# ViktorLiang/GW-Depth

Hardware: AMD Instinct MI355X
Metric: images/sec (train fwd+bwd) 480x640 bs=8/GPU (higher is better)
Workload: dtype bf16; 1 GPU; GW-Depth full model (res50 + DETR 6+6 + 4-scale ReferTransformer + decoder) fwd+17 losses+bwd+clip+AdamW, 480x640, bs=8/GPU, dropout 0.1; global_batch=8, parallelism=dp1, launch=hipgraph, graph_segments=1, grad_buckets=8

## Files before the change

gw_depth_amd/hip.py:

```python
import ctypes
import os

import torch

_HERE = os.path.dirname(os.path.abspath(__file__))
LIB_PATH = os.environ.get("GWD_LIB") or os.path.join(_HERE, "libgwdepth_hip.so")

F32, BF16 = 0, 1
ACT_NONE, ACT_RELU, ACT_GELU, ACT_ELU, ACT_SIGMOID = 0, 1, 2, 3, 4
WS_INORM_GELU, WS_RESAMPLE_BWD, WS_EVAL, WS_PLANE, WS_HEALTH = 0, 1, 2, 3, 4
GATHER_CONV, GATHER_TRANSPOSED, GATHER_UPSAMPLED = 0, 1, 2
RESAMPLE_BILINEAR_AC, RESAMPLE_NEAREST = 0, 1

ENTRY_POINTS = [
    "gwd_version", "gwd_arch", "gwd_conv_forward", "gwd_conv_wgrad", "gwd_weight_prep", "gwd_act_backward",
    "gwd_colsum", "gwd_layernorm_forward", "gwd_layernorm_backward", "gwd_softmax_forward",
    "gwd_softmax_backward", "gwd_silog_sums", "gwd_silog_backward", "gwd_seg_ce_sum", "gwd_seg_ce_backward",
    "gwd_sqnorm", "gwd_adamw_step", "gwd_resample_forward", "gwd_resample_backward", "gwd_avgpool_forward",
    "gwd_avgpool_backward", "gwd_winattn_forward", "gwd_winattn_backward", "gwd_tokattn_forward",
    "gwd_tokattn_backward", "gwd_tokattn_pair_forward", "gwd_tokattn_pair_backward", "gwd_upsample_taps_collapse", "gwd_upsample_taps_fold", "gwd_certain_sample", "gwd_lsap", "gwd_window_map", "gwd_window_map_multi",
    "gwd_inorm_gelu_forward", "gwd_inorm_gelu_backward", "gwd_weight_prep_batch",
    "gwd_point_sample_forward", "gwd_point_sample_backward", "gwd_act_backward_colsum", "gwd_resample_backward_sep",
    "gwd_softmax_masked_forward", "gwd_softmax_scaled_backward", "gwd_query_workspace", "gwd_eval_accumulate", "gwd_colsum_batch", "gwd_conv_wgrad_batch",
    "gwd_conv_wgrad_takes_bias",
    "gwd_plane_loss_forward", "gwd_plane_loss_backward", "gwd_collate",
    "gwd_anchor_depth_forward", "gwd_anchor_depth_backward", "gwd_mha_flash_forward", "gwd_mha_flash_backward",
    "gwd_ref_scores_forward", "gwd_ref_scores_backward", "gwd_ref_mix_forward", "gwd_ref_mix_backward", "gwd_unpad_add_batch", "gwd_stem_pack", "gwd_stem_forward", "gwd_pos_sine", "gwd_silog_finalize", "gwd_psp_pool_forward", "gwd_psp_pool_backward",
    "gwd_match_cost", "gwd_set_losses_forward", "gwd_set_losses_backward", "gwd_set_losses_focal_forward", "gwd_set_losses_focal_backward", "gwd_resample_u8_pass", "gwd_gather2d", "gwd_point_sample_backward_gather", "gwd_point_sample_framed_forward", "gwd_point_sample_framed_backward", "gwd_stride_place", "gwd_color_adjust", "gwd_bmm",
    "gwd_dense_postprocess", "gwd_line_postprocess", "gwd_line_score",
    "gwd_dense_postprocess_resized",
    "gwd_resample_u8_pass_batch", "gwd_gather2d_batch", "gwd_color_adjust_batch",
    "gwd_pyr_tail_forward", "gwd_pyr_tail_backward", "gwd_pyr_tail_fold_wgrad",
    "gwd_widen_u16_batch",
    "gwd_line_nms",
    "gwd_eval_frames",
    "gwd_segment_stats", "gwd_health_decide", "gwd_adamw_step_guarded",
    "gwd_adamw_step_ema", "gwd_ema_swap",
]


class HipUnavailable(RuntimeError):
    pass


class ConvDesc(ctypes.Structure):
    _fields_ = [("x", ctypes.c_void_p), ("w", ctypes.c_void_p), ("y", ctypes.c_void_p), ("z", ctypes.c_void_p),
                ("scale", ctypes.c_void_p), ("shift", ctypes.c_void_p), ("residual", ctypes.c_void_p),
                ("zero_page", ctypes.c_void_p), ("mult", ctypes.c_void_p), ("gate", ctypes.c_void_p)] + \
               [(n, ctypes.c_int32) for n in ("B", "Hi", "Wi", "Cin", "Ho", "Wo", "Cout", "KH", "KW", "stride", "pad",
                                              "gather", "Hv", "Wv", "act")] + \
               [("act_scale", ctypes.c_float), ("dtype", ctypes.c_int32), ("gate_act", ctypes.c_int32),
                ("ln_mean", ctypes.c_void_p), ("ln_rstd", ctypes.c_void_p), ("ln_C", ctypes.c_int32), ("reserved", ctypes.c_int32),
                ("dbias", ctypes.c_void_p)]


class BmmDesc(ctypes.Structure):
    _fields_ = [("a", ctypes.c_void_p), ("b", ctypes.c_void_p), ("c", ctypes.c_void_p)] + \
               [(n, ctypes.c_int64) for n in ("a_sb0", "a_sb1", "a_ld", "b_sb0", "b_sb1", "b_ld", "c_sb0", "c_sb1", "c_ld")] + \
               [(n, ctypes.c_int32) for n in ("M", "N", "K", "nb0", "nb1", "a_kmajor", "b_kmajor", "c_is_f32_accumulate", "splits")] + \
               [("alpha", ctypes.c_float), ("dtype", ctypes.c_int32)]


class PrepJob(ctypes.Structure):
    _fields_ = [("w", ctypes.c_void_p), ("row_scale", ctypes.c_void_p), ("w_fwd", ctypes.c_void_p), ("w_dgrad", ctypes.c_void_p),
                ("N", ctypes.c_int32), ("taps", ctypes.c_int32), ("C", ctypes.c_int32), ("block0", ctypes.c_int32),
                ("Np", ctypes.c_int32), ("Cg", ctypes.c_int32), ("Cgp", ctypes.c_int32), ("reserved", ctypes.c_int32)]


class UnpadJob(ctypes.Structure):
    _fields_ = [("src", ctypes.c_void_p), ("dst", ctypes.c_void_p), ("N", ctypes.c_int32), ("taps", ctypes.c_int32), ("G", ctypes.c_int32),
# ... 145 lines not shown
        L.gwd_set_losses_forward.argtypes = [vp] * 9 + [f32] + [vp] * 4 + [i32] * 6 + [vp]
        L.gwd_set_losses_backward.argtypes = [vp] * 8 + [f32] + [vp] * 6 + [i32] * 6 + [vp]
        L.gwd_set_losses_focal_forward.argtypes = [vp] * 9 + [f32] * 2 + [vp] * 4 + [i32] * 6 + [vp]
        L.gwd_set_losses_focal_backward.argtypes = [vp] * 8 + [f32] * 2 + [vp] * 6 + [i32] * 6 + [vp]
        L.gwd_color_adjust.argtypes = [vp, vp, vp, i64, i32, f32, vp]
        L.gwd_bmm.argtypes = [ctypes.POINTER(BmmDesc), vp]
        L.gwd_stride_place.argtypes = [vp, vp, vp] + [i32] * 8 + [vp]
        L.gwd_psp_pool_forward.argtypes = [vp] * 5 + [i32] * 5 + [vp]
        L.gwd_psp_pool_backward.argtypes = [vp] * 6 + [i32] * 6 + [vp]
        L.gwd_pos_sine.argtypes = [vp, vp, vp, vp, vp, i32, i32, i32, i32, i32, i32, i32, vp]
        L.gwd_stem_pack.argtypes = [vp, vp, vp, vp]
        L.gwd_stem_forward.argtypes = [vp, vp, vp, vp, i32, i32, i32, i32, vp]
        L.gwd_softmax_forward.argtypes = [vp, vp, i64, i32, i32, vp]
        L.gwd_softmax_backward.argtypes = [vp, vp, vp, i64, i32, i32, vp]
        L.gwd_silog_sums.argtypes = [vp, vp, vp, i32, i32, i32, i32, i32, i32, i32, vp]
        L.gwd_silog_backward.argtypes = [vp, vp, vp, vp, f32, f32, vp, i32, i32, i32, i32, i32, i32, i32, vp]
        L.gwd_seg_ce_sum.argtypes = [vp, vp, vp, i64, i32, vp]
        L.gwd_seg_ce_backward.argtypes = [vp, vp, vp, f32, vp, i64, i32, vp]
        L.gwd_resample_forward.argtypes = [vp, vp] + [i32] * 9 + [vp]
        L.gwd_resample_backward.argtypes = [vp, vp] + [i32] * 7 + [vp, i32, i32, vp]
        L.gwd_avgpool_forward.argtypes = [vp, vp] + [i32] * 6 + [vp]
        L.gwd_avgpool_backward.argtypes = [vp, vp] + [i32] * 6 + [vp]
        sp = ctypes.POINTER(Strided)
        L.gwd_winattn_forward.argtypes = [sp, sp, sp, sp, vp, vp, i32, vp, i64, i32, i32, i32, f32, i32, vp]
        L.gwd_winattn_backward.argtypes = [sp] * 7 + [vp, vp, vp, i32, vp, i64, i32, i32, i32, f32, i32, i32, vp]
        L.gwd_ref_scores_forward.argtypes = [sp, vp, vp, i32, i32, i32, i32, i32, f32, i32, vp]
        L.gwd_ref_scores_backward.argtypes = [sp, vp, vp, sp, vp, i32, i32, i32, i32, i32, f32, i32, vp]
        L.gwd_ref_mix_forward.argtypes = [vp, vp, vp, vp, i32, i32, i32, i32, i32, i32, vp]
        L.gwd_ref_mix_backward.argtypes = [vp, vp, vp, vp, vp, i32, i32, i32, i32, i32, i32, vp]
        L.gwd_tokattn_forward.argtypes = [sp] * 4 + [i64, i32, i32, f32, i32, vp]
        L.gwd_tokattn_backward.argtypes = [sp] * 7 + [i64, i32, i32, f32, i32, vp]
        L.gwd_upsample_taps_collapse.argtypes = [vp, vp, i32, i32, i32, vp]
        L.gwd_upsample_taps_fold.argtypes = [vp, vp, i32, i32, vp]
        L.gwd_tokattn_pair_forward.argtypes = [sp] * 6 + [i64, i32, i32, f32, i32, vp]
        L.gwd_tokattn_pair_backward.argtypes = [sp] * 10 + [i64, i32, i32, f32, i32, vp]
        L.gwd_certain_sample.argtypes = [vp, vp, vp, i32, i32, i32, i32, i32, vp, i32, i32, vp]
        L.gwd_lsap.argtypes = [vp, vp, vp, i32, i32, i32, i32, i32, vp]
        L.gwd_inorm_gelu_forward.argtypes = [vp, vp, vp, vp, vp, i64, i64, i32, i32, ctypes.c_float, i32, vp]
        L.gwd_inorm_gelu_backward.argtypes = [vp, vp, vp, vp, vp, i64, i64, i32, i32, i32, vp]
        L.gwd_query_workspace.argtypes = [i32, ctypes.POINTER(ctypes.c_int64), i32]
        L.gwd_query_workspace.restype = ctypes.c_int64
        L.gwd_eval_accumulate.argtypes = [vp, vp, vp, i64, i64, i64, vp, vp, vp, vp, vp, i32, i64, f32, f32, i32, i32, vp]
        L.gwd_dense_postprocess.argtypes = [vp, vp, i64, i64, i64, vp, vp, vp, vp, i32, i32, i32, f32, f32, i32, i32, vp]
        L.gwd_dense_postprocess_resized.argtypes = [vp, vp, i64, i64, i64, vp, vp, i32, vp, vp, vp] + [i32] * 5 + [f32, f32, i32, i32, vp]
        L.gwd_line_postprocess.argtypes = [vp] * 7 + [i32, i32, i32, f32, vp]
        dp = ctypes.POINTER(ctypes.c_double)
        L.gwd_line_score.argtypes = [vp] * 5 + [dp, i32, dp, i32] + [vp] * 4 + [i32] * 4 + [i64, i64, vp]
        L.gwd_softmax_masked_forward.argtypes = [vp, vp, vp, i64, i32, i64, ctypes.c_float, i32, vp]
        L.gwd_softmax_scaled_backward.argtypes = [vp, vp, vp, i64, i32, ctypes.c_float, i32, vp]
        L.gwd_resample_backward_sep.argtypes = [vp, vp, vp] + [i32] * 9 + [vp]
        L.gwd_act_backward_colsum.argtypes = [vp, vp, vp, vp, i64, i32, i32, ctypes.c_float, vp, i32, vp]
        L.gwd_point_sample_forward.argtypes = [vp, vp, vp, i32, i32, i32, i32, i32, i32, i32, vp]
        L.gwd_point_sample_backward.argtypes = [vp, vp, vp, i32, i32, i32, i32, i32, i32, i32, vp]
        L.gwd_point_sample_backward_gather.argtypes = [vp, vp, vp, i32, i32, i32, i32, i32, i32, i32, vp]
        L.gwd_point_sample_framed_forward.argtypes = [vp, vp, vp, i32, i32, i32, i32, i32, i32, i32, i32, i32, vp]
        L.gwd_point_sample_framed_backward.argtypes = [vp, vp, vp, i32, i32, i32, i32, i32, i32, i32, i32, i32, vp]
        L.gwd_weight_prep_batch.argtypes = [vp, i32, i32, vp, vp]
        L.gwd_window_map.argtypes = [vp, vp, vp, i32, i32, i32, i32, i32, i32, i32, vp]
        L.gwd_window_map_multi.argtypes = [vp, vp, vp, vp, i32, i32, i32, i32, i32, i32, i32, vp]
        L.gwd_sqnorm.argtypes = [vp, vp, i64, vp]
        L.gwd_adamw_step.argtypes = [vp, vp, vp, vp, vp, vp, i64] + [f32] * 9 + [vp]
        pvp, pi32 = ctypes.POINTER(ctypes.c_void_p), ctypes.POINTER(ctypes.c_int32)
        L.gwd_pyr_tail_forward.argtypes = [vp, pvp, pi32, pi32, i32] + [vp] * 6 + [i32] * 6 + [vp]
        L.gwd_pyr_tail_backward.argtypes = [vp, pvp, pi32, pi32, i32] + [i32] * 5 + [vp]
        L.gwd_pyr_tail_fold_wgrad.argtypes = [vp, pvp, i32, vp, i32, i32, i32, vp]
        L.gwd_widen_u16_batch.argtypes = [ctypes.POINTER(WidenJob), i32, vp]
# ... 482 lines not shown
                                                 dtype_code(ra), self._stream(ra, ref_v, q_new, att)), "gwd_ref_mix_forward")

    def ref_mix_backward(self, att, ref_v, g, d_ra, d_ref_v, H):
        B, T, R = att.shape[0], att.shape[1], att.shape[2]
        self._check(self.lib.gwd_ref_mix_backward(_ptr(att), _ptr(ref_v), _ptr(g), _ptr(d_ra), _ptr(d_ref_v), B, T, R, H,
                                                  ref_v.shape[2] // H, dtype_code(att), self._stream(att, ref_v, g, d_ra, d_ref_v)),
                    "gwd_ref_mix_backward")

    def tokattn_forward(self, q, k, v, o, scale):
        W, N, H, _ = q.shape
        s = [_strided(t) for t in (q, k, v, o)]
        self._check(self.lib.gwd_tokattn_forward(*[ctypes.byref(x) for x in s], W, H, k.shape[3], scale, dtype_code(q),
                                                 self._stream(q, k, v, o)), "gwd_tokattn_forward")

    def tokattn_backward(self, q, k, v, go, gq, gk, gv, scale):
        W, N, H, _ = q.shape
        s = [_strided(t) for t in (q, k, v, go, gq, gk, gv)]
        self._check(self.lib.gwd_tokattn_backward(*[ctypes.byref(x) for x in s], W, H, k.shape[3], scale, dtype_code(q),
                                                  self._stream(q, go, gq)), "gwd_tokattn_backward")

    def upsample_taps_collapse(self, w, wk):
        Cout, KH, KW, Cin = w.shape
        if (KH, KW) != (3, 3) or tuple(wk.shape) != (Cin, 4, 4, Cout) or w.dtype != torch.float32 or not (w.is_contiguous() and wk.is_contiguous()):
            raise ValueError("upsample_taps_collapse: w (Cout,3,3,Cin) fp32 -> wk (Cin,4,4,Cout), both contiguous")
        self._check(self.lib.gwd_upsample_taps_collapse(_ptr(w), _ptr(wk), Cout, Cin, dtype_code(wk), self._stream(w, wk)), "gwd_upsample_taps_collapse")

    def upsample_taps_fold(self, D, dw):
        Cout, KH, KW, Cin = dw.shape
        if (KH, KW) != (3, 3) or tuple(D.shape) != (Cin, 4, 4, Cout) or D.dtype != torch.float32 or dw.dtype != torch.float32 \
                or not (D.is_contiguous() and dw.is_contiguous()):
            raise ValueError("upsample_taps_fold: D (Cin,4,4,Cout) fp32 -> dw (Cout,3,3,Cin) fp32, both contiguous")
        self._check(self.lib.gwd_upsample_taps_fold(_ptr(D), _ptr(dw), Cout, Cin, self._stream(D, dw)), "gwd_upsample_taps_fold")

    PYR_MAX_BRANCHES = 4

    @staticmethod
    def _pyr_branches(maps, B, N, like):
        if not 1 <= len(maps) <= HipLibrary.PYR_MAX_BRANCHES:
            raise ValueError("pyr_tail: 1 to %d low-resolution branches, got %d" % (HipLibrary.PYR_MAX_BRANCHES, len(maps)))
        for m in maps:
            if m.dim() != 5 or m.shape[0] != B or m.shape[3] != 9 or m.shape[4] != N or m.dtype != like.dtype or not m.is_contiguous():
                raise ValueError("pyr_tail: a product map is (B,h,w,9,N) contiguous in the map's dtype, got %r" % (tuple(m.shape),))
        ptrs = (ctypes.c_void_p * len(maps))(*[m.data_ptr() for m in maps])
        hk = (ctypes.c_int32 * len(maps))(*[m.shape[1] for m in maps])
        wk = (ctypes.c_int32 * len(maps))(*[m.shape[2] for m in maps])
        return ptrs, hk, wk

    def pyr_tail_forward(self, part, Zs, gamma, beta, z, y, mean, rstd, gelu):
        B, H, W, N = part.shape
        ptrs, hk, wk = self._pyr_branches(Zs, B, N, part)
        rc = self.lib.gwd_pyr_tail_forward(_ptr(part), ptrs, hk, wk, len(Zs), _ptr(gamma), _ptr(beta), _ptr(z), _ptr(y), _ptr(mean), _ptr(rstd),
                                           B, H, W, N, int(bool(gelu)), dtype_code(part), self._stream(part, y, *Zs))
        if rc == -4:
            return False
        self._check(rc, "gwd_pyr_tail_forward")
        return True

    def pyr_tail_backward(self, gz, Gs):
        B, H, W, N = gz.shape
        ptrs, hk, wk = self._pyr_branches(Gs, B, N, gz)
        self._check(self.lib.gwd_pyr_tail_backward(_ptr(gz), ptrs, hk, wk, len(Gs), B, H, W, N, dtype_code(gz), self._stream(gz, *Gs)),
                    "gwd_pyr_tail_backward")

    def pyr_tail_fold_wgrad(self, d_hi, d_low, dw, C2):
        N, Cw, nlow = dw.shape[0], dw.shape[-1], len(d_low)
        nbr = Cw // C2 - 1
# ... 309 lines not shown
```

gw_depth_amd/ops.py:

```python
import bisect
import os

import torch
import torch.nn.functional as F

from . import hip
from .hip import (ACT_ELU, ACT_GELU, ACT_NONE, ACT_RELU, ACT_SIGMOID, GATHER_CONV, GATHER_TRANSPOSED,
                  GATHER_UPSAMPLED)

__all__ = ["conv2d", "linear", "layer_norm", "softmax_lastdim", "silog_loss", "seg_cross_entropy",
           "ACT_NONE", "ACT_RELU", "ACT_GELU", "ACT_ELU", "ACT_SIGMOID"]


def _lib():
    return hip.library()


class WeightCache:

    def __init__(self, persistent=(), frozen=False):
        self.frozen = bool(frozen)
        self._derived = {}
        self.ranges = sorted((int(a), int(b)) for a, b in persistent)
        self._starts, self._ends, self._merged_from = [], [], -1
# ... 246 lines not shown
    N, C = w.shape[0], w.shape[-1]
    _lib().weight_prep(w.detach(), row_scale, out, None, N, w.numel() // (N * C), C, hip.F32 if dtype == torch.float32 else hip.BF16)
    return out


def derived_weight(w, tag, make):
    if _ACTIVE_WEIGHTS is not None and _ACTIVE_WEIGHTS.frozen and w.is_cuda and not torch.is_grad_enabled():
        return _ACTIVE_WEIGHTS.derived(w, tag, make)
    return make()


def _weight_transposed(w, row_scale, dtype):
    if dtype == torch.bfloat16 and _ACTIVE_WEIGHTS is not None:
        cached = _ACTIVE_WEIGHTS.get(w, row_scale, "t")
        if cached is not None:
            return cached
    N, C = w.shape[0], w.shape[-1]
    taps = w.numel() // (N * C)
    out = torch.empty((C,) + tuple(w.shape[1:-1]) + (N,), dtype=dtype, device=w.device)
    _lib().weight_prep(w.detach(), row_scale, None, out, N, taps, C, hip.F32 if dtype == torch.float32 else hip.BF16)
    return out


_DIM_T = {}


def _upsampled_dgrad_weight(w, dtype):
    Cout, _, _, Cin = w.shape
    wk = torch.empty((Cin, 4, 4, Cout), dtype=dtype, device=w.device)
    _lib().upsample_taps_collapse(w.detach().float().contiguous(), wk)
    return wk




def mask_levels(pad_mask, sizes):
    lib = _lib()
    B = pad_mask.shape[0]
    full = pad_mask.contiguous().view(torch.uint8) if pad_mask.dtype == torch.bool else pad_mask.contiguous()
    out = []
    for h, w in sizes:
        lvl = torch.empty((B, h, w), dtype=torch.uint8, device=pad_mask.device)
        counts = torch.empty((B, h, w, 2), dtype=torch.int16, device=pad_mask.device)
        lib.pos_counts(full, lvl, counts)
        m = lvl.view(torch.bool)
        m._gwd_counts = counts
        out.append(m)
    return out


def pos_sine(mask, num_pos_feats, normalize, temperature=10000.0):
    counts = mask._gwd_counts
    key = (num_pos_feats, float(temperature), str(mask.device))
    dim_t = _DIM_T.get(key)
    if dim_t is None:
        t = torch.arange(num_pos_feats, dtype=torch.float32, device=mask.device)
        dim_t = _DIM_T[key] = temperature ** (2 * torch.div(t, 2, rounding_mode="floor") / num_pos_feats)
    B, h, w, _ = counts.shape
    out = torch.empty((B, h, w, 2 * num_pos_feats), dtype=torch.float32, device=mask.device)
    _lib().pos_emit(counts, dim_t, out, normalize)
    return out


_STEM_PACKED = {}
_STEM_RETIRED = []

# ... 117 lines not shown
        dims, pad, geom, sink = ctx.cfg
        gx, gw = _conv_backward_stride1(ctx.needs_input_grad[0], ctx.needs_input_grad[1], x, w, gy.contiguous(), g_in, dims, pad, geom, sink)
        return gx, gw, None, None, None, None


def conv2d_padded(x, w, pad, geom, fanout=False):
    return _PadConvFn.apply(x, w, int(pad), tuple(int(v) for v in geom), _sink(w), bool(fanout))


class _ConvFn(torch.autograd.Function):

    @staticmethod
    def forward(ctx, x, w, bias, residual, row_scale, shift_const, stride, pad, act, act_scale, virt, shadow, sinks, mult=None, fanout=False,
                in_gate=ACT_NONE, defer=False, gate_src=None):
        lib = _lib()
        ctx.fan = bool(fanout)
        ctx.in_gate, ctx.defer = int(in_gate), bool(defer)
        if defer and (act not in (ACT_RELU, ACT_ELU, ACT_GELU) or act_scale != 1.0 or mult is not None or (act == ACT_GELU and fanout)):
            raise ValueError("conv2d: defer needs ReLU / ELU / GELU with act_scale 1 and no dropout multiplier")
        if in_gate not in (ACT_NONE, ACT_RELU, ACT_ELU, ACT_GELU) or (in_gate == ACT_GELU) != (gate_src is not None):
            raise ValueError("conv2d: in_gate is ReLU or ELU, or GELU with the producer's pre-activation tensor as gate_src")
        B, Hi, Wi, Cin = x.shape
        Cout, KH, KW, Cw = w.shape
        if Cw != Cin:
            raise ValueError("conv2d: weight expects %d input channels, input has %d" % (Cw, Cin))
        if virt is None:
            Ho = (Hi + 2 * pad - KH) // stride + 1
            Wo = (Wi + 2 * pad - KW) // stride + 1
            gather, vv = GATHER_CONV, (0, 0)
        else:
            Ho, Wo = virt[0] + 2 * pad - KH + 1, virt[1] + 2 * pad - KW + 1
            gather, vv = GATHER_UPSAMPLED, tuple(virt)
        x = x.contiguous()
        wk = _weight_for(w, row_scale, x.dtype, shadow)
        shift = shift_const if bias is None else (bias.detach().float() if shift_const is None else shift_const + bias.detach().float())
        y = torch.empty((B, Ho, Wo, Cout), dtype=x.dtype, device=x.device)
        need_grad = any(ctx.needs_input_grad[:4])
        z = torch.empty_like(y) if (act == ACT_GELU and need_grad) else None
        if residual is not None:
            residual = residual.contiguous()
        dims = (B, Hi, Wi, Cin, Ho, Wo, Cout, KH, KW)
        if mult is not None:
            mult = mult.contiguous()
        lib.conv_forward(x, wk, y, dims, z=z, shift=shift, residual=residual, stride=stride, pad=pad, gather=gather,
                         virt=vv, act=act, act_scale=act_scale, mult=mult)
        ctx.cfg = (dims, stride, pad, act, act_scale, gather, vv, bias is not None, residual is not None)
        ctx.sinks = sinks
        if mult is not None and (act not in (ACT_NONE, ACT_RELU) or (act == ACT_RELU and residual is not None)):
            raise ValueError("conv2d: a dropout multiplier is supported behind no activation (+ skip) or behind ReLU (no skip) only")
        ctx.save_for_backward(x, w, row_scale, z if act == ACT_GELU else (y if act != ACT_NONE else None), mult, gate_src)
        if defer and act == ACT_GELU:
            if z is None:
                z = y
            ctx.mark_non_differentiable(z)
            ctx.set_materialize_grads(False)
            return y, z
        if fanout:
            return y, x.view_as(x)
        return y

    @staticmethod
    def backward(ctx, gy, *g_fan):
        if gy is None:
            return (None,) * 18
        g_in = _fan_in(ctx, g_fan)
        x, w, row_scale, ref, mult, gate_src = ctx.saved_tensors
        dims, stride, pad, act, act_scale, gather, vv, has_bias, has_res = ctx.cfg
        gy = gy.contiguous()
        w_sink, b_sink = ctx.sinks if ctx.sinks is not None else (None, None)
        want_b = has_bias and ctx.needs_input_grad[2]
        dv, bias_done = _conv_act_backward(gy, ref, mult, act, act_scale, ctx.defer, b_sink if want_b else None, dims)
        gx = g_in
        if ctx.needs_input_grad[0]:
            gx = _conv_dgrad(x, w, row_scale, dv, g_in, dims, stride, pad, gather, vv, ctx.in_gate, gate_src)
        gw, gb = _conv_param_grads(x, w, row_scale, dv, dims, stride, pad, gather, vv, ctx.needs_input_grad[1], want_b and not bias_done,
                                   w_sink, b_sink)
        gres = (gy if mult is not None else dv) if (has_res and ctx.needs_input_grad[3]) else None
        return gx, gw, gb, gres, None, None, None, None, None, None, None, None, None, None, None, None, None, None


def _conv_act_backward(gy, ref, mult, act, act_scale, defer, b_sink, dims):
    lib = _lib()
    rows, Cout = dims[0] * dims[4] * dims[5], dims[6]

    def with_colsum(g, dv, m):
        done = lib.act_backward_colsum(g, ref, dv, b_sink[0], rows, Cout, act, act_scale, mult=m)
        if done and b_sink[1] is not None:
            b_sink[1]()
        return done

    if defer:
        return gy, False
    if mult is not None:
        if b_sink is not None:
            dv = torch.empty_like(gy)
            if with_colsum(gy, dv, mult):
                return dv, True
        gy = gy * mult
    if act == ACT_NONE and act_scale == 1.0:
        return gy, False
    dv = torch.empty_like(gy)
    bias_done = b_sink is not None and with_colsum(gy, dv, None)
    if not bias_done:
        lib.act_backward(gy, ref, dv, None, rows, Cout, act, act_scale)
    return dv, bias_done


def _conv_dgrad(x, w, row_scale, dv, g_in, dims, stride, pad, gather, vv, in_gate, gate_src):
    lib = _lib()
    B, Hi, Wi, Cin, Ho, Wo, Cout, KH, KW = dims
    wt = _weight_transposed(w, row_scale, x.dtype)
    gate = dict(gate=(x if gate_src is None else gate_src), gate_act=in_gate) if in_gate != ACT_NONE else {}
    if (gather == GATHER_UPSAMPLED and x.is_cuda and x.dtype == torch.bfloat16 and KH == 3 and KW == 3
            and pad == 1 and vv == (2 * Hi, 2 * Wi) and row_scale is None and (g_in is None or not gate)):
        gx = torch.empty_like(x)
        lib.conv_forward(dv, _upsampled_dgrad_weight(w, x.dtype), gx, (B, Ho, Wo, Cout, Hi, Wi, Cin, 4, 4), stride=2, pad=1,
                         residual=g_in, **gate)
        return gx
    if gather == GATHER_UPSAMPLED:
        gxv = torch.empty((B, vv[0], vv[1], Cin), dtype=x.dtype, device=x.device)
        lib.conv_forward(dv, wt, gxv, (B, Ho, Wo, Cout, vv[0], vv[1], Cin, KH, KW), stride=1, pad=pad, gather=GATHER_TRANSPOSED)
        if gate and g_in is None:
            return _nearest_upsample_backward(gxv, Hi, Wi, gate=x, gate_act=in_gate)
        gx = _nearest_upsample_backward(gxv, Hi, Wi)
        if g_in is not None:
            gx = gx + g_in
        if gate:
            gated = torch.empty_like(gx)
            lib.act_backward(gx, x, gated, None, B * Hi * Wi, Cin, in_gate, 1.0)
            gx = gated
        return gx
    gx = torch.empty_like(x)
    if KH == 1 and KW == 1 and stride > 1 and pad == 0 and not gate:
        q = torch.empty((B, Ho, Wo, Cin), dtype=x.dtype, device=x.device)
        lib.conv_forward(dv, wt, q, (B, Ho, Wo, Cout, Ho, Wo, Cin, 1, 1), stride=1, pad=0, gather=GATHER_TRANSPOSED)
        if lib.stride_place(q, g_in, gx, stride):
            return gx
    if lib.conv_forward(dv, wt, gx, _dgrad_dims(dims), stride=stride, pad=pad, gather=GATHER_TRANSPOSED, residual=g_in, **gate) is False:
        lib.conv_forward(dv, wt, gx, _dgrad_dims(dims), stride=stride, pad=pad, gather=GATHER_TRANSPOSED, residual=g_in)
        gated = torch.empty_like(gx)
        lib.act_backward(gx, gate["gate"], gated, None, B * Hi * Wi, Cin, in_gate, 1.0)
        gx = gated
    return gx


def _conv_param_grads(x, w, row_scale, dv, dims, stride, pad, gather, vv, want_w, want_b, w_sink, b_sink):
    lib = _lib()
    B, Hi, Wi, Cin, Ho, Wo, Cout, KH, KW = dims
    gw = gb = None
    if want_w:
# ... 1300 lines not shown
```

include/gwdepth.h:

```cpp
#ifndef GWDEPTH_H
#define GWDEPTH_H
#include <stdint.h>

#ifdef __cplusplus
extern "C" {
#endif

#define GWD_VERSION 10

enum { GWD_F32 = 0, GWD_BF16 = 1 };
enum { GWD_ACT_NONE = 0, GWD_ACT_RELU = 1, GWD_ACT_GELU = 2, GWD_ACT_ELU = 3, GWD_ACT_SIGMOID = 4 };
enum {
    GWD_GATHER_CONV = 0,
    GWD_GATHER_TRANSPOSED = 1,
    GWD_GATHER_UPSAMPLED = 2
};

typedef struct {
    const void *x;
    const void *w;
    void *y;
    void *z;
    const float *scale;
    const float *shift;
// ... 82 lines not shown

typedef struct {
    void *p;
    int64_t ws, ts, hs;
} gwd_strided;

int gwd_winattn_forward(const gwd_strided *q, const gwd_strided *k, const gwd_strided *v, const gwd_strided *o,
                        const float *bias, const int32_t *rel_index, int32_t n_rel, const int32_t *region, int64_t n_windows,
                        int32_t windows_per_image, int32_t heads, int32_t head_dim, float scale, int32_t dtype, void *stream);
int gwd_winattn_backward(const gwd_strided *q, const gwd_strided *k, const gwd_strided *v, const gwd_strided *go,
                         const gwd_strided *gq, const gwd_strided *gk, const gwd_strided *gv, const float *bias,
                         float *dbias, const int32_t *rel_index, int32_t n_rel, const int32_t *region, int64_t n_windows,
                         int32_t windows_per_image, int32_t heads, int32_t head_dim, float scale, int32_t dbias_head_major,
                         int32_t dtype, void *stream);

int gwd_ref_scores_forward(const gwd_strided *q, const void *ref_k, void *ra, int32_t B, int32_t nwin, int32_t R, int32_t H,
                           int32_t hd, float scale, int32_t dtype, void *stream);
int gwd_ref_scores_backward(const gwd_strided *q, const void *ref_k, const void *g, const gwd_strided *dq, float *d_ref_k, int32_t B,
                            int32_t nwin, int32_t R, int32_t H, int32_t hd, float scale, int32_t dtype, void *stream);
int gwd_ref_mix_forward(const void *ra, const void *ref_v, void *q_new, void *att, int32_t B, int32_t T, int32_t R, int32_t H,
                        int32_t hd, int32_t dtype, void *stream);
int gwd_ref_mix_backward(const void *att, const void *ref_v, const void *g, void *d_ra, float *d_ref_v, int32_t B, int32_t T,
                         int32_t R, int32_t H, int32_t hd, int32_t dtype, void *stream);

int gwd_tokattn_forward(const gwd_strided *q, const gwd_strided *k, const gwd_strided *v, const gwd_strided *o,
                        int64_t n_windows, int32_t heads, int32_t e, float scale, int32_t dtype, void *stream);
int gwd_tokattn_backward(const gwd_strided *q, const gwd_strided *k, const gwd_strided *v, const gwd_strided *go,
                         const gwd_strided *gq, const gwd_strided *gk, const gwd_strided *gv, int64_t n_windows,
                         int32_t heads, int32_t e, float scale, int32_t dtype, void *stream);

int gwd_upsample_taps_collapse(const float *w, void *wk, int32_t Cout, int32_t Cin, int32_t dtype, void *stream);
int gwd_upsample_taps_fold(const float *D, float *dw, int32_t Cout, int32_t Cin, void *stream);

int gwd_tokattn_pair_forward(const gwd_strided *q, const gwd_strided *q2, const gwd_strided *k, const gwd_strided *v,
                             const gwd_strided *o, const gwd_strided *o2, int64_t n_windows, int32_t heads, int32_t e,
                             float scale, int32_t dtype, void *stream);
int gwd_tokattn_pair_backward(const gwd_strided *q, const gwd_strided *q2, const gwd_strided *k, const gwd_strided *v,
                              const gwd_strided *go, const gwd_strided *go2, const gwd_strided *gq, const gwd_strided *gq2,
                              const gwd_strided *gk, const gwd_strided *gv, int64_t n_windows, int32_t heads, int32_t e,
                              float scale, int32_t dtype, void *stream);

int gwd_certain_sample(const float *pred_small, const float *pred_large, float *coords, int32_t B, int32_t hs,
                       int32_t ws, int32_t H, int32_t W, const float *edges, int32_t n_intervals,
                       int32_t sample_num, void *stream);

int gwd_lsap(const float *cost, const int32_t *col_offsets, int32_t *query_of_target, int32_t layers, int32_t B,
             int32_t Q, int32_t sum_targets, int32_t max_targets, void *stream);

int gwd_point_sample_forward(const void *map, const float *coords, float *out, int32_t B, int32_t H, int32_t W, int32_t C,
                             int32_t S, int32_t mode, int32_t dtype, void *stream);
int gwd_point_sample_backward(const float *gout, const float *coords, void *gmap, int32_t B, int32_t H, int32_t W, int32_t C,
                              int32_t S, int32_t mode, int32_t dtype, void *stream);
int gwd_point_sample_backward_gather(const float *gout, const float *coords, void *gmap, int32_t B, int32_t H, int32_t W, int32_t C,
                                     int32_t S, int32_t mode, int32_t dtype, void *stream);

int gwd_point_sample_framed_forward(const void *map, const float *coords, float *out, int32_t B, int32_t H, int32_t W, int32_t C,
                                    int32_t S, int32_t Hf, int32_t Wf, int32_t shift, int32_t dtype, void *stream);
int gwd_point_sample_framed_backward(const float *gout, const float *coords, void *gmap, int32_t B, int32_t H, int32_t W, int32_t C,
                                     int32_t S, int32_t Hf, int32_t Wf, int32_t shift, int32_t dtype, void *stream);

typedef struct gwd_prep_job {
    const float *w;
    const float *row_scale;
    void *w_fwd;
    void *w_dgrad;
    int32_t N, taps, C;
// ... 250 lines not shown
```

Measured before the change: 260.6 images/s.

## Add collapsed-weight subpixel kernel for nearest-upsample 3x3 convs

Adds a dedicated HIP kernel for a 3x3 conv applied to a 2x nearest-upsampled input. It folds the 3x3 weights into four 2x2 sub-pixel kernels, one per output phase, so each output needs 4 taps instead of 9 and reads the low-resolution input directly from an LDS halo tile using MFMA. The same collapse pass also produces the 4x4 dgrad weight, which is stored on ctx and reused in backward instead of being rebuilt. Routing applies only to the (64,64) and (64,32) channel pairs above a pixel threshold, and falls back to the generic conv otherwise. The cost is an extra per-step weight-collapse kernel, since the dgrad operands are not cached.

```diff
diff --git a/gw_depth_amd/csrc/upconv.hip b/gw_depth_amd/csrc/upconv.hip
--- /dev/null
+++ b/gw_depth_amd/csrc/upconv.hip
@@ -0,0 +1,223 @@
+#include "common.h"
+
+namespace upconv {
+
+constexpr int TILE_H = 4;
+constexpr int TW = 32, HW = TW + 2;
+
+typedef __attribute__((ext_vector_type(4))) unsigned u32x4;
+
+__device__ __forceinline__ f32x16 mma(const bf16x8 &a, const bf16x8 &b, const f32x16 &c) {
+    return __builtin_amdgcn_mfma_f32_32x32x16_bf16(a, b, c, 0, 0, 0);
+}
+
+typedef __attribute__((ext_vector_type(2))) float f32x2;
+typedef __attribute__((ext_vector_type(2))) __bf16 bf16x2;
+
+__device__ __forceinline__ f32x2 elu2(f32x2 v) {
+    const f32x2 m = {fminf(v.x, 0.f), fminf(v.y, 0.f)}, t = m * 1.44269504f;
+    const f32x2 e = {__builtin_amdgcn_exp2f(t.x), __builtin_amdgcn_exp2f(t.y)}, p = {fmaxf(v.x, 0.f), fmaxf(v.y, 0.f)};
+    return p + (e - 1.0f);
+}
+template <int ACTK> __device__ __forceinline__ f32x2 act_out(f32x2 v, int act) {
+    if constexpr (ACTK == GWD_ACT_ELU) return elu2(v);
+    else return f32x2{apply_act(v.x, ACTK < 0 ? act : ACTK), apply_act(v.y, ACTK < 0 ? act : ACTK)};
+}
+
+template <int CIN, int TH> struct Halo {
+    static constexpr int HPIX = (TH + 2) * HW, NT = 64 * TH;
+    static constexpr int PS = CIN + 8;
+    static constexpr int CHUNKS = HPIX * (CIN / 8);
+    static constexpr int NCH = (CHUNKS + NT - 1) / NT;
+};
+
+template <int CIN, int TH>
+__device__ __forceinline__ u32x4 halo_fetch(const __bf16 *__restrict__ x, int chunk, int b, int y0, int x0, int Hi, int Wi) {
+    const u32x4 z = {0u, 0u, 0u, 0u};
+    if (chunk >= Halo<CIN, TH>::CHUNKS) return z;
+    const int hp = chunk / (CIN / 8), part = chunk - hp * (CIN / 8);
+    const int hy = hp / HW, hx = hp - hy * HW;
+    const int sy = y0 - 1 + hy, sx = x0 - 1 + hx;
+    if ((unsigned)sy >= (unsigned)Hi || (unsigned)sx >= (unsigned)Wi) return z;
+    return *(const u32x4 *)(x + (((size_t)b * Hi + sy) * Wi + sx) * CIN + part * 8);
+}
+
+template <int CIN, int COUT, int TH, int ACTK>
+__global__ __launch_bounds__(64 * TH, 2) void upconv_fwd_kernel(const gwd_conv_desc d, int tiles_y, int tiles_x, int ntiles) {
+    using H = Halo<CIN, TH>;
+    constexpr int NT = H::NT, HPIX = H::HPIX;
+    constexpr int NTL = COUT / 32, KS = CIN / 16;
+    constexpr int RB = NTL == 1 ? 2 : 1;
+    __shared__ __attribute__((aligned(16))) __bf16 halo[HPIX * H::PS];
+    __shared__ __attribute__((aligned(16))) float shl[COUT];
+    const int tid = threadIdx.x, lane = tid & 63, wave = tid >> 6, r = lane & 31, h = lane >> 5;
+    const int cls = wave & 3, py = cls >> 1, px = cls & 1, grp = wave >> 2;
+    const __bf16 *x = (const __bf16 *)d.x, *w = (const __bf16 *)d.w;
+    __bf16 *y = (__bf16 *)d.y;
+    const int Hi = d.Hi, Wi = d.Wi, Hv = 2 * d.Hi, Wv = 2 * d.Wi;
+    if (tid < COUT) shl[tid] = d.shift ? d.shift[tid] : 0.f;
+
+    bf16x8 wa[4][NTL][KS];
+#pragma unroll
+    for (int tap = 0; tap < 4; ++tap)
+#pragma unroll
+        for (int nt = 0; nt < NTL; ++nt)
+#pragma unroll
+            for (int s = 0; s < KS; ++s)
+                wa[tap][nt][s] = *(const bf16x8 *)(w + ((size_t)((cls * 4 + tap) * COUT + 32 * nt + r)) * CIN + 16 * s + 8 * h);
+
+    u32x4 pre[H::NCH];
+    int tile = blockIdx.x;
+    auto where = [&](int t, int &b, int &y0, int &x0) {
+        const int per = tiles_y * tiles_x;
+        b = t / per;
+        const int rem = t - b * per;
+        y0 = (rem / tiles_x) * TH;
+        x0 = (rem % tiles_x) * TW;
+    };
+    if (tile < ntiles) {
+        int b, y0, x0;
+        where(tile, b, y0, x0);
+#pragma unroll
+        for (int i = 0; i < H::NCH; ++i) pre[i] = halo_fetch<CIN, TH>(x, tid + NT * i, b, y0, x0, Hi, Wi);
+    }
+    for (; tile < ntiles; tile += gridDim.x) {
+        int b, y0, x0;
+        where(tile, b, y0, x0);
+        __syncthreads();
+#pragma unroll
+        for (int i = 0; i < H::NCH; ++i) {
+            const int chunk = tid + NT * i;
+            if (chunk < H::CHUNKS) *(u32x4 *)(halo + (chunk / (CIN / 8)) * H::PS + (chunk % (CIN / 8)) * 8) = pre[i];
+        }
+        __syncthreads();
+        if (tile + (int)gridDim.x < ntiles) {
+            int nb, ny, nx;
+            where(tile + gridDim.x, nb, ny, nx);
+#pragma unroll
+            for (int i = 0; i < H::NCH; ++i) pre[i] = halo_fetch<CIN, TH>(x, tid + NT * i, nb, ny, nx, Hi, Wi);
+        }
+#pragma unroll 1
+        for (int rc = 0; rc < 4; rc += RB) {
+            const int yl = 4 * grp + rc;
+            if (y0 + yl >= Hi) break;
+            f32x16 acc[RB][NTL];
+#pragma unroll
+            for (int m = 0; m < RB; ++m)
+#pragma unroll
+                for (int nt = 0; nt < NTL; ++nt)
+#pragma unroll
+                    for (int i = 0; i < 16; ++i) acc[m][nt][i] = 0.f;
+            bf16x8 bf[2][KS][RB];
+            auto fetch = [&](int buf, int tap) {
+                const int a = tap >> 1, bq = tap & 1;
+#pragma unroll
+                for (int s = 0; s < KS; ++s)
+#pragma unroll
+                    for (int m = 0; m < RB; ++m)
+                        bf[buf][s][m] = *(const bf16x8 *)(halo + ((yl + m + py + a) * HW + r + px + bq) * H::PS + 16 * s + 8 * h);
+            };
+            constexpr bool AHEAD = NTL == 1;
+            if constexpr (AHEAD) fetch(0, 0);
+#pragma unroll
+            for (int tap = 0; tap < 4; ++tap) {
+                if constexpr (AHEAD) {
+                    if (tap < 3) fetch((tap + 1) & 1, tap + 1);
+                    __builtin_amdgcn_sched_barrier(0);
+                } else
+                    fetch(tap & 1, tap);
+#pragma unroll
+                for (int s = 0; s < KS; ++s)
+#pragma unroll
+                    for (int nt = 0; nt < NTL; ++nt)
+#pragma unroll
+                        for (int m = 0; m < RB; ++m) acc[m][nt] = mma(wa[tap][nt][s], bf[tap & 1][s][m], acc[m][nt]);
+            }
+#pragma unroll
+            for (int m = 0; m < RB; ++m) {
+                const int ly = y0 + yl + m, lx = x0 + r;
+                const bool inside = ly < Hi && lx < Wi;
+                __bf16 *dst = y + (((size_t)b * Hv + 2 * ly + py) * Wv + 2 * lx + px) * COUT;
+#pragma unroll
+                for (int nt = 0; nt < NTL; ++nt)
+#pragma unroll
+                    for (int k = 0; k < 2; ++k) {
+                        union { unsigned u[2]; bf16x2 e[2]; } v[2];
+#pragma unroll
+                        for (int q = 0; q < 2; ++q) {
+                            const int g = 2 * k + q;
+                            const f32x4 sh = *(const f32x4 *)(shl + 32 * nt + 8 * g + 4 * h);
+#pragma unroll
+                            for (int j = 0; j < 2; ++j) {
+                                const f32x2 pre2 = f32x2{acc[m][nt][4 * g + 2 * j], acc[m][nt][4 * g + 2 * j + 1]} + f32x2{sh[2 * j], sh[2 * j + 1]};
+                                v[q].e[j] = __builtin_convertvector(act_out<ACTK>(pre2, d.act) * d.act_scale, bf16x2);
+                            }
+                        }
+                        const auto s0 = __builtin_amdgcn_permlane32_swap(v[0].u[0], v[1].u[0], false, false);
+                        const auto s1 = __builtin_amdgcn_permlane32_swap(v[0].u[1], v[1].u[1], false, false);
+                        if (inside) *(u32x4 *)(dst + 32 * nt + 8 * (2 * k + h)) = u32x4{s0[0], s1[0], s0[1], s1[1]};
+                    }
+            }
+        }
+    }
+}
+
+template <int CIN, int COUT>
+int launch(const gwd_conv_desc *d, int max_workgroups, hipStream_t s) {
+    constexpr int TH = TILE_H, NT = 64 * TH;
+    const int ty = (d->Hi + TH - 1) / TH, tx = (d->Wi + TW - 1) / TW;
+    const long ntiles = (long)d->B * ty * tx;
+    long grid = 256L * (8 / TH);
+    if (max_workgroups > 0 && grid > max_workgroups) grid = max_workgroups;
+    if (grid > ntiles) grid = ntiles;
+    if (d->act == GWD_ACT_NONE)
+        upconv_fwd_kernel<CIN, COUT, TH, GWD_ACT_NONE><<<(unsigned)grid, NT, 0, s>>>(*d, ty, tx, (int)ntiles);
+    else if (d->act == GWD_ACT_ELU)
+        upconv_fwd_kernel<CIN, COUT, TH, GWD_ACT_ELU><<<(unsigned)grid, NT, 0, s>>>(*d, ty, tx, (int)ntiles);
+    else
+        upconv_fwd_kernel<CIN, COUT, TH, -1><<<(unsigned)grid, NT, 0, s>>>(*d, ty, tx, (int)ntiles);
+    GWD_CHECK_LAUNCH();
+    return 0;
+}
+
+__global__ void collapse_kernel(const float *__restrict__ w, __bf16 *__restrict__ wf, __bf16 *__restrict__ wk, int Cout, int Cin) {
+    const int total = Cin * 16 * Cout;
+    for (int i = blockIdx.x * blockDim.x + threadIdx.x; i < total; i += gridDim.x * blockDim.x) {
+        const int co = i % Cout, ts = (i / Cout) & 15, ci = i / (16 * Cout);
+        const int t = ts >> 2, s = ts & 3;
+        float acc = 0.f;
+        for (int kh = max(0, 2 - t); kh <= min(2, 3 - t); ++kh)
+            for (int kw = max(0, 2 - s); kw <= min(2, 3 - s); ++kw) acc += w[((size_t)(co * 3 + kh) * 3 + kw) * Cin + ci];
+        const __bf16 v = (__bf16)acc;
+        if (wk) wk[i] = v;
+        const int py = (3 - t) & 1, a = (3 - t) >> 1, px = (3 - s) & 1, b = (3 - s) >> 1;
+        wf[((size_t)(((py * 2 + px) * 2 + a) * 2 + b) * Cout + co) * Cin + ci] = v;
+    }
+}
+
+}
+
+extern "C" int gwd_upconv_collapse(const float *w, void *w_fwd, void *w_dgrad, int32_t Cout, int32_t Cin, void *stream) {
+    if (!w || !w_fwd || Cout <= 0 || Cin <= 0 || (int64_t)Cout * Cin * 16 > INT32_MAX) return -1;
+    const int total = Cin * 16 * Cout;
+    int blocks = (total + 255) / 256;
+    if (blocks > 1024) blocks = 1024;
+    upconv::collapse_kernel<<<blocks, 256, 0, (hipStream_t)stream>>>(w, (__bf16 *)w_fwd, (__bf16 *)w_dgrad, Cout, Cin);
+    GWD_CHECK_LAUNCH();
+    return 0;
+}
+
+extern "C" int gwd_upconv_forward(const gwd_conv_desc *d, int32_t max_workgroups, void *stream) {
+    if (!d || !d->x || !d->y || !d->w) return -1;
+    if (d->dtype != GWD_BF16) return -2;
+    if (d->B <= 0 || d->Hi <= 0 || d->Wi <= 0 || d->Cin <= 0 || d->Ho <= 0 || d->Wo <= 0 || d->Cout <= 0) return -3;
+    if (d->KH != 3 || d->KW != 3 || d->stride != 1 || d->pad != 1 || max_workgroups < 0) return -4;
+    if (d->residual || d->gate || d->z || d->mult || d->scale || d->ln_mean || d->ln_rstd) return -4;
+    if (d->gather != GWD_GATHER_UPSAMPLED) return -5;
+    if (d->Hv != 2 * (int64_t)d->Hi || d->Wv != 2 * (int64_t)d->Wi || d->Ho != d->Hv || d->Wo != d->Wv) return -6;
+    if ((int64_t)d->B * d->Ho * d->Wo >= (1LL << 31)) return -7;
+    if (((uintptr_t)d->x | (uintptr_t)d->w | (uintptr_t)d->y) % 16 || (uintptr_t)d->shift % 4) return -8;
+    if (d->Cin == 64 && d->Cout == 64) return upconv::launch<64, 64>(d, max_workgroups, (hipStream_t)stream);
+    if (d->Cin == 64 && d->Cout == 32) return upconv::launch<64, 32>(d, max_workgroups, (hipStream_t)stream);
+    return -4;
+}
diff --git a/gw_depth_amd/hip.py b/gw_depth_amd/hip.py
--- a/gw_depth_amd/hip.py
+++ b/gw_depth_amd/hip.py
@@ -36,6 +36,7 @@
     "gwd_eval_frames",
     "gwd_segment_stats", "gwd_health_decide", "gwd_adamw_step_guarded",
     "gwd_adamw_step_ema", "gwd_ema_swap",
+    "gwd_upconv_collapse", "gwd_upconv_forward",
 ]
 
 
@@ -247,6 +248,8 @@
         L.gwd_tokattn_backward.argtypes = [sp] * 7 + [i64, i32, i32, f32, i32, vp]
         L.gwd_upsample_taps_collapse.argtypes = [vp, vp, i32, i32, i32, vp]
         L.gwd_upsample_taps_fold.argtypes = [vp, vp, i32, i32, vp]
+        L.gwd_upconv_collapse.argtypes = [vp, vp, vp, i32, i32, vp]
+        L.gwd_upconv_forward.argtypes = [ctypes.POINTER(ConvDesc), i32, vp]
         L.gwd_tokattn_pair_forward.argtypes = [sp] * 6 + [i64, i32, i32, f32, i32, vp]
         L.gwd_tokattn_pair_backward.argtypes = [sp] * 10 + [i64, i32, i32, f32, i32, vp]
         L.gwd_certain_sample.argtypes = [vp, vp, vp, i32, i32, i32, i32, i32, vp, i32, i32, vp]
@@ -795,6 +798,18 @@
             raise ValueError("upsample_taps_fold: D (Cin,4,4,Cout) fp32 -> dw (Cout,3,3,Cin) fp32, both contiguous")
         self._check(self.lib.gwd_upsample_taps_fold(_ptr(D), _ptr(dw), Cout, Cin, self._stream(D, dw)), "gwd_upsample_taps_fold")
 
+    def upconv_collapse(self, w, w_fwd, w_dgrad=None):
+        Cout, KH, KW, Cin = w.shape
+        if (KH, KW) != (3, 3) or tuple(w_fwd.shape) != (2, 2, 2, 2, Cout, Cin) or w.dtype != torch.float32 or w_fwd.dtype != torch.bfloat16 \
+                or not (w.is_contiguous() and w_fwd.is_contiguous()) \
+                or (w_dgrad is not None and (tuple(w_dgrad.shape) != (Cin, 4, 4, Cout) or w_dgrad.dtype != torch.bfloat16 or not w_dgrad.is_contiguous())):
+            raise ValueError("upconv_collapse: w (Cout,3,3,Cin) fp32 -> w_fwd (2,2,2,2,Cout,Cin) [, w_dgrad (Cin,4,4,Cout)] bf16, all contiguous")
+        self._check(self.lib.gwd_upconv_collapse(_ptr(w), _ptr(w_fwd), _ptr(w_dgrad), Cout, Cin, self._stream(w, w_fwd, w_dgrad)), "gwd_upconv_collapse")
+
+    def upconv_forward(self, x, w_fwd, y, dims, max_workgroups=0, **kw):
+        d = self._desc(x, w_fwd, y, dims, **kw)
+        return self.lib.gwd_upconv_forward(ctypes.byref(d), int(max_workgroups), self._stream(x, w_fwd, y))
+
     PYR_MAX_BRANCHES = 4
 
     @staticmethod
diff --git a/gw_depth_amd/ops.py b/gw_depth_amd/ops.py
--- a/gw_depth_amd/ops.py
+++ b/gw_depth_amd/ops.py
@@ -302,6 +302,23 @@
     return wk
 
 
+UPCONV_COLLAPSED = True
+UPCONV_COLLAPSED_MIN_PIXELS = 131072
+UPCONV_COLLAPSED_PAIRS = ((64, 64), (64, 32))
+
+
+def _upconv_operands(w, want_dgrad):
+    Cout, _, _, Cin = w.shape
+
+    def make(dg=None):
+        wf = torch.empty((2, 2, 2, 2, Cout, Cin), dtype=torch.bfloat16, device=w.device)
+        _lib().upconv_collapse(w.detach().float().contiguous(), wf, dg)
+        return wf
+
+    if want_dgrad:
+        dg = torch.empty((Cin, 4, 4, Cout), dtype=torch.bfloat16, device=w.device)
+        return make(dg), dg
+    return derived_weight(w, "upconv_fwd", make), None
 
 
 def mask_levels(pad_mask, sizes):
@@ -485,7 +502,6 @@
             Ho, Wo = virt[0] + 2 * pad - KH + 1, virt[1] + 2 * pad - KW + 1
             gather, vv = GATHER_UPSAMPLED, tuple(virt)
         x = x.contiguous()
-        wk = _weight_for(w, row_scale, x.dtype, shadow)
         shift = shift_const if bias is None else (bias.detach().float() if shift_const is None else shift_const + bias.detach().float())
         y = torch.empty((B, Ho, Wo, Cout), dtype=x.dtype, device=x.device)
         need_grad = any(ctx.needs_input_grad[:4])
@@ -495,8 +511,21 @@
         dims = (B, Hi, Wi, Cin, Ho, Wo, Cout, KH, KW)
         if mult is not None:
             mult = mult.contiguous()
-        lib.conv_forward(x, wk, y, dims, z=z, shift=shift, residual=residual, stride=stride, pad=pad, gather=gather,
-                         virt=vv, act=act, act_scale=act_scale, mult=mult)
+        ctx.up_wk = None
+        routed = False
+        if (UPCONV_COLLAPSED and gather == GATHER_UPSAMPLED and x.is_cuda and x.dtype == torch.bfloat16 and w.dtype == torch.float32
+                and (KH, KW, stride, pad) == (3, 3, 1, 1) and vv == (2 * Hi, 2 * Wi) and (Cin, Cout) in UPCONV_COLLAPSED_PAIRS
+                and residual is None and mult is None and row_scale is None and act != ACT_GELU
+                and B * Ho * Wo >= UPCONV_COLLAPSED_MIN_PIXELS):
+            wf, dg = _upconv_operands(w, ctx.needs_input_grad[0])
+            routed = lib.upconv_forward(x, wf, y, dims, shift=shift, stride=stride, pad=pad, gather=gather, virt=vv, act=act,
+                                        act_scale=act_scale) == 0
+            if routed:
+                ctx.up_wk = dg
+        if not routed:
+            wk = _weight_for(w, row_scale, x.dtype, shadow)
+            lib.conv_forward(x, wk, y, dims, z=z, shift=shift, residual=residual, stride=stride, pad=pad, gather=gather,
+                             virt=vv, act=act, act_scale=act_scale, mult=mult)
         ctx.cfg = (dims, stride, pad, act, act_scale, gather, vv, bias is not None, residual is not None)
         ctx.sinks = sinks
         if mult is not None and (act not in (ACT_NONE, ACT_RELU) or (act == ACT_RELU and residual is not None)):
@@ -525,7 +554,7 @@
         dv, bias_done = _conv_act_backward(gy, ref, mult, act, act_scale, ctx.defer, b_sink if want_b else None, dims)
         gx = g_in
         if ctx.needs_input_grad[0]:
-            gx = _conv_dgrad(x, w, row_scale, dv, g_in, dims, stride, pad, gather, vv, ctx.in_gate, gate_src)
+            gx = _conv_dgrad(x, w, row_scale, dv, g_in, dims, stride, pad, gather, vv, ctx.in_gate, gate_src, ctx.up_wk)
         gw, gb = _conv_param_grads(x, w, row_scale, dv, dims, stride, pad, gather, vv, ctx.needs_input_grad[1], want_b and not bias_done,
                                    w_sink, b_sink)
         gres = (gy if mult is not None else dv) if (has_res and ctx.needs_input_grad[3]) else None
@@ -559,7 +588,7 @@
     return dv, bias_done
 
 
-def _conv_dgrad(x, w, row_scale, dv, g_in, dims, stride, pad, gather, vv, in_gate, gate_src):
+def _conv_dgrad(x, w, row_scale, dv, g_in, dims, stride, pad, gather, vv, in_gate, gate_src, up_wk=None):
     lib = _lib()
     B, Hi, Wi, Cin, Ho, Wo, Cout, KH, KW = dims
     wt = _weight_transposed(w, row_scale, x.dtype)
@@ -567,8 +596,8 @@
     if (gather == GATHER_UPSAMPLED and x.is_cuda and x.dtype == torch.bfloat16 and KH == 3 and KW == 3
             and pad == 1 and vv == (2 * Hi, 2 * Wi) and row_scale is None and (g_in is None or not gate)):
         gx = torch.empty_like(x)
-        lib.conv_forward(dv, _upsampled_dgrad_weight(w, x.dtype), gx, (B, Ho, Wo, Cout, Hi, Wi, Cin, 4, 4), stride=2, pad=1,
-                         residual=g_in, **gate)
+        lib.conv_forward(dv, up_wk if up_wk is not None else _upsampled_dgrad_weight(w, x.dtype), gx, (B, Ho, Wo, Cout, Hi, Wi, Cin, 4, 4),
+                         stride=2, pad=1, residual=g_in, **gate)
         return gx
     if gather == GATHER_UPSAMPLED:
         gxv = torch.empty((B, vv[0], vv[1], Cin), dtype=x.dtype, device=x.device)
diff --git a/include/gwdepth.h b/include/gwdepth.h
--- a/include/gwdepth.h
+++ b/include/gwdepth.h
@@ -138,6 +138,9 @@
 int gwd_upsample_taps_collapse(const float *w, void *wk, int32_t Cout, int32_t Cin, int32_t dtype, void *stream);
 int gwd_upsample_taps_fold(const float *D, float *dw, int32_t Cout, int32_t Cin, void *stream);
 
+int gwd_upconv_collapse(const float *w, void *w_fwd, void *w_dgrad, int32_t Cout, int32_t Cin, void *stream);
+int gwd_upconv_forward(const gwd_conv_desc *d, int32_t max_workgroups, void *stream);
+
 int gwd_tokattn_pair_forward(const gwd_strided *q, const gwd_strided *q2, const gwd_strided *k, const gwd_strided *v,
                              const gwd_strided *o, const gwd_strided *o2, int64_t n_windows, int32_t heads, int32_t e,
                              float scale, int32_t dtype, void *stream);
```

Result: no change. 262.4 images/s (median of 6 runs) (+0.7%).
